# opencb/hpg-variant

Measured on AMD Instinct MI355X. Metric: variants/s chi2 assoc, higher is better.
Workload: dtype u8

## Files before the change

hpg-variant_amd/csrc/hpgv_capi.hip:

```cpp
#include "hpgv_internal.h"
#include <cstdlib>

extern "C" {

const char *hpgv_version(void) { return "hpgv-mi355x 0.1 (gfx950)"; }

int hpgv_device_count(void) {
    int n = 0;
    if (hipGetDeviceCount(&n) != hipSuccess) return -1;
    return n;
}

const char *hpgv_last_error(const hpgv_ctx *ctx) { return ctx ? ctx->err.c_str() : g_create_error.c_str(); }

static void read_environment(hpgv_ctx *ctx) {
    auto num = [](const char *name, long lo, long hi, long *out) { const char *e = getenv(name); if (e && *e) { long v = atol(e); *out = v < lo ? lo : v > hi ? hi : v; } };
    num("HPGV_BATCH_COPY", 0, 1, &ctx->batch_copy);
    num("HPGV_BATCH_FUSED", 0, 1, &ctx->batch_fused);
    num("HPGV_STATS_ALL2", 0, 1, &ctx->stats_all2);
    num("HPGV_ASSOC_ROWS", 0, 1, &ctx->assoc_rows);
    num("HPGV_PINNED_NONCOHERENT", 0, 1, &ctx->pinned_noncoherent);
    num("HPGV_VMM_TRACE", 0, 1, &ctx->vmm_trace);
    num("HPGV_DECODE_TILES", 0, 1, &ctx->decode_tiles);
#ifdef HPGV_ABLATION
// ... 45 lines not shown
        return rc;
    }
    *out = ctx;
    return HPGV_OK;
}

int hpgv_create_multi(const int *device_ids, int n_devices, hpgv_ctx **out) {
    if (!out) return fail(nullptr, HPGV_ERR_INVALID, "out is NULL");
    *out = nullptr;
    if (!device_ids || n_devices < 1 || n_devices > 64) return fail(nullptr, HPGV_ERR_INVALID, "hpgv_create_multi needs 1..64 device ids");
    hpgv_ctx *g = new (std::nothrow) hpgv_ctx();
    if (!g) return fail(nullptr, HPGV_ERR_NOMEM, "out of host memory");
    for (int i = 0; i < n_devices; ++i) {
        hpgv_ctx *m = nullptr;
        const int rc = hpgv_create(device_ids[i], &m);
        if (rc != HPGV_OK) {
            for (hpgv_ctx *c : g->members) { c->parent = nullptr; hpgv_destroy(c); }
            g->members.clear();
            delete g;
            return rc;
        }
        m->parent = g;
        g->members.push_back(m);
    }
    g->device = g->members[0]->device;
    *out = g;
    return HPGV_OK;
}

int hpgv_group_size(const hpgv_ctx *ctx) { return !ctx ? 0 : (is_group(ctx) ? (int)ctx->members.size() : 1); }

hpgv_ctx *hpgv_group_member(hpgv_ctx *ctx, int i) {
    if (!ctx) return nullptr;
    if (!is_group(ctx)) return i == 0 ? ctx : nullptr;
    return (i >= 0 && i < (int)ctx->members.size()) ? ctx->members[(size_t)i] : nullptr;
}

int hpgv_member_device(const hpgv_ctx *ctx, int i) {
    if (!ctx) return -1;
    if (!is_group(ctx)) return i == 0 ? ctx->device : -1;
    return (i >= 0 && i < (int)ctx->members.size()) ? ctx->members[(size_t)i]->device : -1;
}

}
namespace {
void grow_release(hpgv_ctx::GrowRange &r) {
    size_t off = 0;
    for (size_t i = 0; i < r.pieces.size(); ++i) { (void)hipMemUnmap(r.base + off, r.sizes[i]); (void)hipMemRelease(r.pieces[i]); off += r.sizes[i]; }
    if (r.base) (void)hipMemAddressFree(r.base, r.reserved);
    r = hpgv_ctx::GrowRange();
}
}
extern "C" {

void hpgv_destroy(hpgv_ctx *ctx) {
    if (!ctx) return;
    if (is_group(ctx)) {
        hpgv_group_release(ctx);
        for (hpgv_ctx *m : ctx->members) { m->parent = nullptr; hpgv_destroy(m); }
        ctx->members.clear();
        delete ctx;
        return;
    }
    DeviceGuard g(ctx->device);
    (void)hipDeviceSynchronize();
    if (ctx->d_mendel_male) (void)hipFree(ctx->d_mendel_male);
    if (ctx->d_sg_chunks) (void)hipFree(ctx->d_sg_chunks);
    if (ctx->d_group_of_col) (void)hipFree(ctx->d_group_of_col);
    if (ctx->d_cond) (void)hipFree(ctx->d_cond);
    for (Layout *L : {&ctx->assoc, &ctx->tdt, &ctx->stats, &ctx->sgroups, &ctx->mendel})
        if (L->d_col_of_pos) (void)hipFree(L->d_col_of_pos);
    ctx->tdt_plan.release();
    if (ctx->d_lf_base) (void)hipFree(ctx->d_lf_base);
    if (ctx->d_thr) (void)hipFree(ctx->d_thr);
    if (ctx->d_sink) (void)hipFree(ctx->d_sink);
    if (ctx->d_crc_tab) (void)hipFree(ctx->d_crc_tab);
    for (auto *t : ctx->tok_scratch) {
        if (t->d_blocks) (void)hipFree(t->d_blocks);
        if (t->d_line_off) (void)hipFree(t->d_line_off);
        if (t->d_extra) (void)hipFree(t->d_extra);
        delete t;
    }
    ctx->tok_scratch.clear();
    for (auto &r : ctx->grow) grow_release(r);
    ctx->grow.clear();
    hpgv_epi_release(ctx->epi);
    for (Slot *s : ctx->slots) {
        for (int i = 0; i < 8; ++i) if (s->buf[i]) (void)hipFree(s->buf[i]);
        if (s->h_res) (void)hipHostFree(s->h_res);
        if (s->cnt_buf) (void)hipFree(s->cnt_buf);
        if (s->stream) (void)hipStreamDestroy(s->stream);
        delete s;
    }
    for (int i = 0; i < 4; ++i) if (ctx->ev[i]) (void)hipEventDestroy(ctx->ev[i]);
    delete ctx;
}

#ifdef HPGV_ABLATION
#define HPGV_SHIPPED_ONLY(ok, what)
#else
#define HPGV_SHIPPED_ONLY(ok, what) if (!(ok)) return fail(ctx, HPGV_ERR_UNSUPPORTED, what ": that form is an ablation build's (-DHPGV_ABLATION, tools/build_ablation.py)");
#endif

int hpgv_set_option(hpgv_ctx *ctx, const char *key, long value) {
    if (is_group(ctx) && key && !strcmp(key, "group_self_exchange")) { ctx->group_self_exchange = value ? 1 : 0; return HPGV_OK; }
    GROUP_ALL(ctx, hpgv_set_option(m_, key, value))
    if (!ctx || !key) return HPGV_ERR_INVALID;
    if (!strcmp(key, "row_align")) {
        if (value < 16 || (value & (value - 1))) return fail(ctx, HPGV_ERR_INVALID, "row_align must be a power of two >= 16");
        if (ctx->assoc.set || ctx->tdt.set || ctx->stats.set)
            return fail(ctx, HPGV_ERR_STATE, "row_align must be set before the cohort");
        ctx->row_align = value;
    } else if (!strcmp(key, "row_pad")) {
        if (value < 0 || value % 16 || value > 65536) return fail(ctx, HPGV_ERR_INVALID, "row_pad must be a multiple of 16 in [0, 65536]");
        if (ctx->assoc.set || ctx->tdt.set || ctx->stats.set)
            return fail(ctx, HPGV_ERR_STATE, "row_pad must be set before the cohort");
        ctx->row_pad = value;
    } else if (!strcmp(key, "variants_per_wave")) {
        if (value < 1 || value > 1024) return fail(ctx, HPGV_ERR_INVALID, "variants_per_wave out of range");
        ctx->vpw = value;
    } else if (!strcmp(key, "nontemporal")) {
        HPGV_SHIPPED_ONLY(value != 0, "nontemporal = 0")
        ctx->nontemporal = value ? 1 : 0;
    } else if (!strcmp(key, "profile")) {
        ctx->profile = value ? 1 : 0;
    } else if (!strcmp(key, "scan_unroll")) {
        if (value != 4 && value != 8 && value != 10 && value != 12 && value != 16)
            return fail(ctx, HPGV_ERR_INVALID, "scan_unroll must be one of 4, 8, 10, 12, 16");
        HPGV_SHIPPED_ONLY(value == 4, "scan_unroll other than 4")
        ctx->scan_unroll = value;
    } else if (!strcmp(key, "pipeline")) {
        HPGV_SHIPPED_ONLY(value != 0, "pipeline = 0")
        ctx->pipeline = value ? 1 : 0;
    } else if (!strcmp(key, "fisher_cut_exp")) {
        if (value < 12 || value > 300) return fail(ctx, HPGV_ERR_INVALID, "fisher_cut_exp must be in [12, 300]");
        ctx->fisher_cut_exp = value;
    } else if (!strcmp(key, "epi_complete")) {
        ctx->epi_complete = value ? 1 : 0;
    } else if (!strcmp(key, "epi_triples_mfma")) {
        ctx->epi_triples_mfma = value ? 1 : 0;
    } else if (!strcmp(key, "epi_pairs_mfma")) {
        ctx->epi_pairs_mfma = value ? 1 : 0;
    } else if (!strcmp(key, "epi_triples_1pass")) {
        if (value < 0 || value > 2) return fail(ctx, HPGV_ERR_INVALID, "epi_triples_1pass must be 0 (two passes), 1 (the cells nine at a time) or 2 (one pass, one wave per SIMD)");
        HPGV_SHIPPED_ONLY(value != 2, "epi_triples_1pass = 2")
        ctx->epi_triples_1pass = value;
    } else if (!strcmp(key, "scan_lds")) {
        if (value < 0 || value > 160 * 1024) return fail(ctx, HPGV_ERR_INVALID, "scan_lds must be in [0, 163840]");
        ctx->scan_lds = value;
    } else if (!strcmp(key, "batch_copy")) {
        ctx->batch_copy = value ? 1 : 0;
    } else if (!strcmp(key, "inflate_wave")) {
        if (value < 0 || value > 4) return fail(ctx, HPGV_ERR_INVALID, "inflate_wave must be 0 (lane per block), 1 (by the number of blocks), 2 (wave per block), 4 (wave per block, several symbols per round) or 3 (lane per block, symbol tables in LDS)");
        HPGV_SHIPPED_ONLY(value == 1 || value == 4, "inflate_wave other than 1 / 4 (a wave per block, several symbols per round)")
        ctx->inflate_wave = value;
    } else if (!strcmp(key, "tokenizer_tiles")) {
        if (value < 0 || value > 2) return fail(ctx, HPGV_ERR_INVALID, "tokenizer_tiles must be 2 (one sweep), 1 (two sweeps) or 0 (line by line)");
        HPGV_SHIPPED_ONLY(value == 1, "tokenizer_tiles other than 1 (two sweeps)")
        ctx->tokenizer_tiles = value;
    } else if (!strcmp(key, "fisher_width")) {
        if (value != 64 && value != 32 && value != 16 && value != 8) return fail(ctx, HPGV_ERR_INVALID, "fisher_width must be 64, 32, 16 or 8");
        HPGV_SHIPPED_ONLY(value == 16, "fisher_width other than 16")
        ctx->fisher_width = value;
    } else if (!strcmp(key, "batch_fused")) {
        ctx->batch_fused = value ? 1 : 0;
    } else if (!strcmp(key, "pipe_waves")) {
        if (value != 4 && value != 6 && value != 8) return fail(ctx, HPGV_ERR_INVALID, "pipe_waves must be 4, 6 or 8");
        HPGV_SHIPPED_ONLY(value == 4, "pipe_waves other than 4")
        ctx->pipe_waves = value;
    } else if (!strcmp(key, "persistent")) {
        HPGV_SHIPPED_ONLY(value == 0, "persistent = 1")
        ctx->persistent = value ? 1 : 0;
    } else if (!strcmp(key, "part_aligned_loads")) {
        HPGV_SHIPPED_ONLY(value == 0, "part_aligned_loads = 1")
        ctx->part_aligned = value ? 1 : 0;
    } else if (!strcmp(key, "blocks_per_cu")) {
        if (value < 1 || value > 8) return fail(ctx, HPGV_ERR_INVALID, "blocks_per_cu must be in 1..8");
        ctx->blocks_per_cu = value;
    } else {
        return fail(ctx, HPGV_ERR_INVALID, "unknown option '%s'", key);
    }
    return HPGV_OK;
}


int hpgv_set_cohort(hpgv_ctx *ctx, const uint8_t *condition, int n_samples) {
    HPGV_ABI_TRY
    GROUP_ALL(ctx, hpgv_set_cohort(m_, condition, n_samples))
    if (!ctx) return HPGV_ERR_INVALID;
    if (!condition || n_samples < 0) return fail(ctx, HPGV_ERR_INVALID, "bad cohort arguments");
    DeviceGuard g(ctx->device);
    int nA = 0, nU = 0;
    for (int j = 0; j < n_samples; ++j) {
        if (condition[j] == HPGV_COND_AFFECTED) nA++;
        else if (condition[j] == HPGV_COND_UNAFFECTED) nU++;
    }
    size_t segA = round_up((size_t)nA, 16), segU = round_up((size_t)nU, 16);
    size_t pitch = round_up(segA + segU, (size_t)ctx->row_align) + (size_t)ctx->row_pad;
    if (pitch == 0) pitch = (size_t)ctx->row_align;
    if (!pitch_supported(pitch)) return fail(ctx, HPGV_ERR_UNSUPPORTED, "cohort of %d samples exceeds the row-length limit", n_samples);
    Layout &L = ctx->assoc;
    L.n_samples = n_samples;
    L.pitch = pitch;
    L.col_of_pos.assign(pitch, -1);
    size_t a = 0, u = segA;
    for (int j = 0; j < n_samples; ++j) {
        if (condition[j] == HPGV_COND_AFFECTED) L.col_of_pos[a++] = j;
        else if (condition[j] == HPGV_COND_UNAFFECTED) L.col_of_pos[u++] = j;
    }
    ctx->nA = nA; ctx->nU = nU; ctx->chunksA = (int)(segA / 16);
    {
        std::vector<uint8_t> cond(round_up((size_t)n_samples, 16) + 16, (uint8_t)HPGV_COND_OTHER);
        for (int j = 0; j < n_samples; ++j) cond[(size_t)j] = condition[j] == HPGV_COND_AFFECTED ? 1 : condition[j] == HPGV_COND_UNAFFECTED ? 0 : 2;
        if (ctx->cond_cap < cond.size()) {
            if (ctx->d_cond) { (void)hipFree(ctx->d_cond); ctx->d_cond = nullptr; ctx->cond_cap = 0; }
            HIPCHK(ctx, hipMalloc(&ctx->d_cond, cond.size()));
            ctx->cond_cap = cond.size();
        }
        HIPCHK(ctx, hipMemcpy(ctx->d_cond, cond.data(), cond.size(), hipMemcpyHostToDevice));
    }
    return upload_layout(ctx, L);
    HPGV_ABI_CATCH(ctx)
}

int hpgv_assoc_layout(const hpgv_ctx *ctx, int *n_affected, int *n_unaffected, size_t *pitch) {
    ctx = first_member(ctx);
    if (!ctx) return HPGV_ERR_INVALID;
    if (!ctx->assoc.set) return fail(ctx, HPGV_ERR_STATE, "hpgv_set_cohort has not been called");
    if (n_affected) *n_affected = ctx->nA;
    if (n_unaffected) *n_unaffected = ctx->nU;
    if (pitch) *pitch = ctx->assoc.pitch;
    return HPGV_OK;
}

int hpgv_set_logfact(hpgv_ctx *ctx, const double *table, size_t n) {
    GROUP_ALL(ctx, hpgv_set_logfact(m_, table, n))
    if (!ctx) return HPGV_ERR_INVALID;
    if (!table || n == 0) return fail(ctx, HPGV_ERR_INVALID, "empty log-factorial table");
    DeviceGuard g(ctx->device);
    ctx->n_lf = 0;
    if (ctx->cap_lf < n) {
        if (ctx->d_lf_base) { (void)hipFree(ctx->d_lf_base); ctx->d_lf_base = nullptr; ctx->d_lf = nullptr; ctx->cap_lf = 0; }
        HIPCHK(ctx, hipMalloc(&ctx->d_lf_base, (n + 4) * sizeof(double)));
        HIPCHK(ctx, hipMemset(ctx->d_lf_base, 0, (n + 4) * sizeof(double)));
        ctx->d_lf = ctx->d_lf_base + 2;
        ctx->cap_lf = n;
// ... 427 lines not shown
```

hpg-variant_amd/csrc/hpgv_internal.h:

```cpp
#pragma once
#include "../../include/hpgv.h"
#include "hpgv_kernels.h"
#include "hpgv_tdt_stats_kernels.h"
#include "hpgv_epi_kernels.h"

#include <hip/hip_runtime.h>
#include <cctype>

#include <algorithm>
#include <atomic>
#include <cmath>
#include <cstdarg>
#include <cstdio>
#include <cstring>
#include <mutex>
#include <new>
#include <string>
#include <vector>

namespace { thread_local std::string g_create_error; }

struct Layout {
    bool set = false;
    int n_samples = 0;
// ... 5 lines not shown
};

struct Slot {
    bool busy = false;
    hipStream_t stream = nullptr;
    void *buf[8] = {nullptr, nullptr, nullptr, nullptr, nullptr, nullptr, nullptr, nullptr};
    size_t cap[8] = {0, 0, 0, 0, 0, 0, 0, 0};
    void *h_res = nullptr;
    void *d_res = nullptr;
    size_t res_cap = 0;
    void *cnt_buf = nullptr;
    size_t cnt_cap = 0;
};

struct Staged {
    const uint8_t *d_raw = nullptr;
    size_t raw_pitch = 0;
    const uint8_t *d_laid = nullptr;
    int which = 0;
    const uint8_t *d_isx = nullptr;
    int n = 0;
    size_t out_stride = 0;
    bool text = false;
};

struct EpiState {
    bool have_data = false, have_folds = false;
    int V = 0, nA = 0, nU = 0, num_folds = 0, W = 0, V_alloc = 0, n_chunks = 0;
    uint8_t *d_data = nullptr;
    uint32_t *d_planes = nullptr;
    uint32_t rev_off = 0;
    hpgv_epi_rank_info rank_info{};
    uint32_t *d_marg = nullptr;
    bool complete = false;
    hpgv::EpiChunk *d_chunks = nullptr;
    uint32_t *d_chunk_cls = nullptr;
    hpgv::EpiFold *d_folds = nullptr;
    uint32_t *d_group_w0 = nullptr;
    std::vector<int32_t> group_size;
    hpgv::EpiCand *d_cand = nullptr;
    hpgv::EpiCand3 *d_cand3 = nullptr;
    size_t cand3_cap = 0;
    unsigned *d_cand_count = nullptr;
    unsigned cand_cap = 0;
    double *d_thr = nullptr;
    unsigned *d_tile_base = nullptr;
    size_t tile_base_cap = 0;
};

struct hpgv_ctx {
    std::vector<hpgv_ctx *> members;
    hpgv_ctx *parent = nullptr;
    struct GroupState *grp = nullptr;
    long group_self_exchange = 0;
    std::atomic<unsigned> deal_next{0};
    std::atomic<int> in_flight{0};
    int device = 0;
    mutable std::string err;
    std::mutex mu;
    long row_align = 16;
    long row_pad = 0;
    long vpw = 2;
    long nontemporal = 1;
    long profile = 0;
    std::mutex alias_mu;
    std::vector<std::pair<const char *, const char *>> text_alias;
    struct TextTiles { const char *d_text, *d_base; const void *d_tiles; uint64_t n_tiles; };
    std::vector<TextTiles> text_tiles;
    struct TextHeld { const char *host_text; Slot *slot; const char *d_text; const unsigned long long *d_line_off; int n_lines; };
    std::vector<TextHeld> text_held;
    long part_aligned = 0;
    long scan_unroll = 4;
    long persistent = 0;
    long blocks_per_cu = 8;
    long pipeline = 1;
    long pipe_waves = 4;
    long fisher_cut_exp = 22;
    long epi_complete = 1;
    long epi_pairs_mfma = 1;
    long epi_triples_mfma = 1;
    long epi_triples_1pass = 1;
    long scan_lds = 0;
    long fisher_width = 16;
    long inflate_wave = 1;
    long tokenizer_tiles = 1;
    long batch_copy = 0;
    long batch_fused = 1;
    long batch_lds_max = 65536;
    long stats_all2 = 1;
    long assoc_rows = 1;
    long pinned_noncoherent = 0;
    long vmm_trace = 0;
    long decode_tiles = 1;
#ifdef HPGV_ABLATION
    long stats_rows = 0, stats_bs = 0, stats_debug = 0;
    long fisher_lds = 0;
    long inflate_lds_pad = 0, inflate_wave_wgs = 0, inflate_lane_wgs = 0;
#endif
    int n_cus = 256;
    Layout assoc;
    int nA = 0, nU = 0, chunksA = 0;
    uint8_t *d_cond = nullptr;
    size_t cond_cap = 0;
    Layout tdt;
    hpgv::TdtPlan tdt_plan;
    Layout stats;
    Layout sgroups;
    std::vector<uint32_t> sg_off;
    std::vector<int> sg_size;
    int32_t *d_sg_chunks = nullptr;
    size_t sg_chunks_cap = 0;
    uint8_t *d_group_of_col = nullptr;
    size_t group_of_col_cap = 0;
    bool all_grouped = false;
    Layout mendel;
    int mendel_trios = 0, mendel_pchunks = 0;
    hpgv::MendelLuts mendel_luts{};
    uint8_t *d_mendel_male = nullptr;
    double *d_lf = nullptr;
    double *d_lf_base = nullptr;
    size_t n_lf = 0;
    size_t cap_lf = 0;
    uint32_t *d_thr = nullptr;
    size_t thr_cap = 0;
    hipEvent_t ev[4] = {nullptr, nullptr, nullptr, nullptr};
    bool have_scan_ev = false, have_stats_ev = false;
    std::vector<Slot *> slots;
    uint32_t *d_sink = nullptr;
    uint32_t *d_crc_tab = nullptr;
    struct TokScratch {
        hipStream_t stream = nullptr;
        int *d_blocks = nullptr; size_t blocks_cap = 0;
        unsigned long long *d_line_off = nullptr; size_t line_cap = 0;
        void *d_extra = nullptr; size_t extra_cap = 0;
    };
    std::mutex tok_mu;
    std::vector<TokScratch *> tok_scratch;
    struct GrowRange { char *base = nullptr; size_t reserved = 0, committed = 0; std::vector<hipMemGenericAllocationHandle_t> pieces; std::vector<size_t> sizes; };
    std::vector<GrowRange> grow;
    double filt_min_maf = -1.0, filt_max_missing = -1.0;
    long filt_max_mendel = -1;
    double filt_min_dom = -1.0, filt_min_rec = -1.0;
    std::mutex epi_mu;
    EpiState epi;
};

namespace {

[[maybe_unused]] int fail(const hpgv_ctx *ctx, int code, const char *fmt, ...) {
    char buf[512];
    va_list ap;
    va_start(ap, fmt);
    vsnprintf(buf, sizeof buf, fmt, ap);
    va_end(ap);
    if (ctx) {
        ctx->err = buf;
        if (ctx->parent) {
            std::lock_guard<std::mutex> lk(ctx->parent->mu);
            ctx->parent->err = buf;
        }
    } else g_create_error = buf;
    return code;
}

#define HPGV_ABI_TRY try {
#define HPGV_ABI_CATCH(ctx)                                                                         \
    } catch (const std::bad_alloc &) { return fail(ctx, HPGV_ERR_NOMEM, "out of host memory"); }     \
      catch (...) { return fail(ctx, HPGV_ERR_INVALID, "unexpected C++ exception inside the engine"); }

inline bool is_group(const hpgv_ctx *c) { return c && !c->members.empty(); }
inline hpgv_ctx *first_member(hpgv_ctx *c) { return is_group(c) ? c->members[0] : c; }
inline const hpgv_ctx *first_member(const hpgv_ctx *c) { return is_group(c) ? c->members[0] : c; }
struct Dealt {
    hpgv_ctx *m;
    explicit Dealt(hpgv_ctx *g) {
        const unsigned n = (unsigned)g->members.size(), start = g->deal_next.fetch_add(1u, std::memory_order_relaxed) % n;
        m = g->members[start];
        int best = m->in_flight.load(std::memory_order_relaxed);
        for (unsigned k = 1; k < n && best > 0; ++k) {
            hpgv_ctx *c = g->members[(start + k) % n];
            const int f = c->in_flight.load(std::memory_order_relaxed);
            if (f < best) { best = f; m = c; }
        }
        m->in_flight.fetch_add(1, std::memory_order_relaxed);
    }
    ~Dealt() { m->in_flight.fetch_sub(1, std::memory_order_relaxed); }
};
#define GROUP_ALL(ctx, CALL)                                                                \
    if (is_group(ctx)) {                                                                    \
        for (hpgv_ctx *m_ : (ctx)->members) { const int rc_ = CALL; if (rc_) return rc_; }  \
        return HPGV_OK;                                                                     \
    }
#define GROUP_DEAL(ctx, CALL)                                                               \
    if (is_group(ctx)) { Dealt d_(ctx); hpgv_ctx *m_ = d_.m; return CALL; }
#define GROUP_DEAL_TEXT(ctx, text, CALL)                                                    \
    if (is_group(ctx)) {                                                                    \
        if (hpgv_ctx *m_ = alias_owner(ctx, text)) return CALL;                             \
        Dealt d_(ctx); hpgv_ctx *m_ = d_.m; return CALL;                                    \
    }

#define HIPCHK(ctx, call)                                                                   \
    do {                                                                                    \
        hipError_t e_ = (call);                                                             \
        if (e_ != hipSuccess)                                                               \
            return fail(ctx, HPGV_ERR_HIP, "%s failed: %s (%s:%d)", #call,                  \
                        hipGetErrorString(e_), __FILE__, __LINE__);                         \
    } while (0)

struct DeviceGuard {
    int prev = -1;
    bool changed = false;
    explicit DeviceGuard(int dev) {
        if (hipGetDevice(&prev) == hipSuccess && prev != dev) {
            changed = (hipSetDevice(dev) == hipSuccess);
        }
    }
    ~DeviceGuard() { if (changed) (void)hipSetDevice(prev); }
};

[[maybe_unused]] size_t round_up(size_t x, size_t a) { return (x + a - 1) / a * a; }
// ... 99 lines not shown
```

hpg-variant_amd/csrc/hpgv_kernels.h:

```cpp
#pragma once
#include <hip/hip_runtime.h>
#include <stdint.h>

namespace hpgv {

__device__ __forceinline__ uint32_t nib_nonzero(uint32_t x) {
    uint32_t y = x | (x << 1);
    y = y | (y << 2);
    return y & 0x88888888u;
}
__device__ __forceinline__ uint32_t nib_not_f(uint32_t x) { return nib_nonzero(~x); }

__device__ __forceinline__ int wave_sum(int v) {
    v += __builtin_amdgcn_update_dpp(0, v, 0xB1, 0xF, 0xF, true);
    v += __builtin_amdgcn_update_dpp(0, v, 0x4E, 0xF, 0xF, true);
    v += __builtin_amdgcn_update_dpp(0, v, 0x141, 0xF, 0xF, true);
    v += __builtin_amdgcn_update_dpp(0, v, 0x140, 0xF, 0xF, true);
    return __builtin_amdgcn_readlane(v, 0) + __builtin_amdgcn_readlane(v, 16) +
           __builtin_amdgcn_readlane(v, 32) + __builtin_amdgcn_readlane(v, 48);
}

template <bool NT>
__device__ __forceinline__ uint4 load16(const uint4 *p);
template <bool NT>
// ... 280 lines not shown
}
template <int W> __device__ __forceinline__ double sub_sum_f64(double v) {
#pragma unroll
    for (int off = W / 2; off > 0; off >>= 1) v += __shfl_xor(v, off);
    return v;
}
template <int W> __device__ __forceinline__ double sub_first_f64(double v, int lane) { return __shfl(v, lane & ~(W - 1)); }

template <int W>
__device__ __forceinline__ void fisher_boundaries(const FisherTab &T, double thr , int L1, int R1, int L2, int R2, int lane,
                                                  int *xL, int *xR) {
    const int sl = sub_lane<W>(lane);
    while (R1 - L1 > W || R2 - L2 > W) {
        const bool go1 = R1 - L1 > W, go2 = R2 - L2 > W;
        const int step1 = (R1 - L1 + W - 1) / W, step2 = (R2 - L2 + W - 1) / W;
        const int x1 = L1 + sl * step1, x2 = L2 + sl * step2;
        const double v1 = (go1 && x1 < R1) ? T.e(x1) : 0.0;
        const double v2 = (go2 && x2 < R2) ? T.e(x2) : 0.0;
        if (go1) {
            const int j = __builtin_popcountll(sub_ballot<W>(x1 < R1 && v1 <= thr, lane));
            const int xj = L1 + j * step1;
            const int nL = (j == 0) ? L1 : L1 + (j - 1) * step1 + 1, nR = (j == W || xj >= R1) ? R1 : xj;
            L1 = nL; R1 = nR;
        }
        if (go2) {
            const int j = __builtin_popcountll(sub_ballot<W>(x2 < R2 && v2 > thr, lane));
            const int xj = L2 + j * step2;
            const int nL = (j == 0) ? L2 : L2 + (j - 1) * step2 + 1, nR = (j == W || xj >= R2) ? R2 : xj;
            L2 = nL; R2 = nR;
        }
    }
    const int x1 = L1 + sl, x2 = L2 + sl;
    const double v1 = x1 < R1 ? T.e(x1) : 0.0, v2 = x2 < R2 ? T.e(x2) : 0.0;
    *xL = L1 + __builtin_popcountll(sub_ballot<W>(x1 < R1 && v1 <= thr, lane));
    *xR = L2 + __builtin_popcountll(sub_ballot<W>(x2 < R2 && v2 > thr, lane));
}

template <int W>
__device__ __forceinline__ double fisher_tails(const FisherTab &T, int xL, int xR, int lo, int hi, int lane, double rel_cut) {
    const int sl = sub_lane<W>(lane);
    double partL = 0.0, partR = 0.0, cutL = 0.0, cutR = 0.0;
    bool onL = true, onR = true;
    for (int k = 0; onL || onR; ++k) {
        const int firstL = xL - 1 - 2 * W * k, firstR = xR + 2 * W * k;
        if (firstL < lo) onL = false;
        if (firstR > hi) onR = false;
        const int a = firstL - 2 * sl, b = firstR + 2 * sl;
        double eL0 = -2000.0, eL1 = -2000.0, eR0 = -2000.0, eR1 = -2000.0;
        if (onL && a >= lo) { double lo_e, hi_e; T.e2(a - 1, &lo_e, &hi_e); eL0 = hi_e; if (a - 1 >= lo) eL1 = lo_e; }
        if (onR && b <= hi) { double lo_e, hi_e; T.e2(b, &lo_e, &hi_e); eR0 = lo_e; if (b + 1 <= hi) eR1 = hi_e; }
        const double sL0 = fisher_exp(eL0, T.xt), sL1 = fisher_exp(eL1, T.xt), sR0 = fisher_exp(eR0, T.xt), sR1 = fisher_exp(eR1, T.xt);
        partL += sL0 + sL1; partR += sR0 + sR1;
        if (k == 0) { cutL = rel_cut * sub_first_f64<W>(sL0, lane); cutR = rel_cut * sub_first_f64<W>(sR0, lane); }
        if (onL && sub_ballot<W>(sL0 > cutL || sL1 > cutL, lane) == 0ull) onL = false;
        if (onR && sub_ballot<W>(sR0 > cutR || sR1 > cutR, lane) == 0ull) onR = false;
    }
    return sub_sum_f64<W>(partL + partR);
}

template <int W>
__device__ __forceinline__ bool fisher_boundary_windows(const FisherTab &T, double thr , int mode, int obs, int lane,
                                                        int *L1, int *R1, int *L2, int *R2) {
    const int sl = sub_lane<W>(lane);
    const int g1 = obs <= mode ? obs + 1 : 2 * mode - obs + 1, g2 = obs <= mode ? 2 * mode - obs : obs;
    int w1 = g1 - W / 2, w2 = g2 - W / 2;
    w1 = w1 > *R1 - W ? *R1 - W : w1; w1 = w1 < *L1 ? *L1 : w1;
    w2 = w2 > *R2 - W ? *R2 - W : w2; w2 = w2 < *L2 ? *L2 : w2;
    const int x1 = w1 + sl, x2 = w2 + sl;
    const bool in1 = x1 < *R1, in2 = x2 < *R2;
    const double v1 = in1 ? T.e(x1) : 0.0, v2 = in2 ? T.e(x2) : 0.0;
    const int n1 = __builtin_popcountll(sub_ballot<W>(in1, lane)), n2 = __builtin_popcountll(sub_ballot<W>(in2, lane));
    const int c1 = __builtin_popcountll(sub_ballot<W>(in1 && v1 <= thr, lane)), c2 = __builtin_popcountll(sub_ballot<W>(in2 && v2 > thr, lane));
    bool ok = true;
    if (c1 == 0 && w1 > *L1) { *R1 = w1; ok = false; }
    else if (c1 == n1 && w1 + n1 < *R1) { *L1 = w1 + n1; ok = false; }
    else { *L1 = w1 + c1; *R1 = w1 + c1; }
    if (c2 == 0 && w2 > *L2) { *R2 = w2; ok = false; }
    else if (c2 == n2 && w2 + n2 < *R2) { *L2 = w2 + n2; ok = false; }
    else { *L2 = w2 + c2; *R2 = w2 + c2; }
    return ok;
}

template <int W>
__device__ __forceinline__ double fisher_sub(int a, int b, int c, int d, const double *__restrict__ lf,
                                             const double *exp_tab , double rel_cut, int lane) {
    const int sl = sub_lane<W>(lane);
    const int r1 = a + b, r2 = c + d, c1 = a + c, nn = r1 + r2;
    const int lo = (c1 - r2) > 0 ? (c1 - r2) : 0;
    const int hi = r1 < c1 ? r1 : c1;
    FisherTab T;
    T.lf = lf; T.xt = exp_tab; T.r1 = r1; T.c1 = c1; T.d0 = r2 - c1;
    T.konst = lf[r1] + lf[r2] + lf[c1] + lf[nn - c1] - lf[nn];
    const double thr = T.e(a) + 9.9999995000000333e-08;
    double sum;
    if (hi - lo < 8 * W) {
        double part = 0.0;
        for (int x = lo + sl; x <= hi; x += W) {
            const double ex = T.e(x);
            if (ex <= thr) part += fisher_exp(ex, exp_tab);
        }
        sum = sub_sum_f64<W>(part);
    } else {
        const double prod = (double)(r1 + 1) * (double)(c1 + 1), den = (double)(nn + 2);
        double md = __builtin_floor(prod / den);
        const double rem = __builtin_fma(-md, den, prod);
        md += rem >= den ? 1.0 : (rem < 0.0 ? -1.0 : 0.0);
        int mode = (int)md;
        mode = mode < lo ? lo : (mode > hi ? hi : mode);
        int L1 = lo, R1 = mode + 1, L2 = mode + 1, R2 = hi + 1, xL, xR;
        if (fisher_boundary_windows<W>(T, thr, mode, a, lane, &L1, &R1, &L2, &R2)) { xL = L1; xR = L2; }
        else fisher_boundaries<W>(T, thr, L1, R1, L2, R2, lane, &xL, &xR);
        sum = fisher_tails<W>(T, xL, xR, lo, hi, lane, rel_cut);
    }
    return sum > 1.0 ? 1.0 : sum;
}

__device__ __forceinline__ double fisher_wave(int a, int b, int c, int d, const double *__restrict__ lf,
                                              const double *exp_tab , double rel_cut, int lane) {
    return fisher_sub<64>(a, b, c, d, lf, exp_tab, rel_cut, lane);
}

template <int W>
__global__ __launch_bounds__(256) void k_assoc_fisher(const int4 *__restrict__ counts, int n,
                                                      const double *__restrict__ lf,
                                                      double *__restrict__ odds,
                                                      double *__restrict__ pval, double rel_cut) {
    __shared__ double exp_tab[64];
    if (threadIdx.x < 64) exp_tab[threadIdx.x] = k_exp2_j64[threadIdx.x];
    __syncthreads();
    const int lane = threadIdx.x & 63;
    constexpr int PER_WAVE = 64 / W;
    const long wave = (long)blockIdx.x * (blockDim.x >> 6) + (threadIdx.x >> 6);
    const long v = wave * PER_WAVE + lane / W;
    if (v >= n) return;
    const int4 c4 = counts[v];
    const int a = c4.x, b = c4.y, c = c4.z, d = c4.w;
    const double p = fisher_sub<W>(a, b, c, d, lf, exp_tab, rel_cut, lane);
    if (sub_lane<W>(lane) == 0) {
        odds[v] = assoc_odds(a, b, c, d);
        pval[v] = p;
    }
}

__host__ __device__ __forceinline__ uint64_t splitmix64(uint64_t x) {
    x ^= x >> 30; x *= 0xbf58476d1ce4e5b9ULL;
    x ^= x >> 27; x *= 0x94d049bb133111ebULL;
    x ^= x >> 31;
    return x;
}
#define HPGV_SYNTH_SEED 0x4850475631ULL

static __global__ void k_synth_thresholds(uint64_t v0, int n, uint32_t *__restrict__ thr) {
    const int i = blockIdx.x * blockDim.x + threadIdx.x;
    if (i >= n) return;
    const uint64_t v = v0 + (uint64_t)i;
    const uint64_t h = splitmix64(HPGV_SYNTH_SEED ^ 0xA11E1EULL ^ v);
    const double u = (double)(h >> 11) * (1.0 / 9007199254740992.0);
    const double q = 0.05 + 0.45 * u;
    const uint32_t t_miss = 167772u;
    const double rest = (double)(16777216u - t_miss);
    const double omq = 1.0 - q;
    const double p00 = omq * omq;
    const double p01 = 2.0 * q * omq;
    const uint32_t t00 = t_miss + (uint32_t)floor(p00 * rest);
    const uint32_t t01 = t00 + (uint32_t)floor(p01 * rest);
    thr[3 * i + 0] = t_miss; thr[3 * i + 1] = t00; thr[3 * i + 2] = t01;
}

__device__ __forceinline__ uint32_t synth_gt(uint64_t vterm, uint64_t s, uint32_t tm, uint32_t t0,
                                             uint32_t t1) {
    const uint32_t r = (uint32_t)(splitmix64(vterm + s) >> 40);
    return (r < tm) ? 0xFFu : (r < t0) ? 0x00u : (r < t1) ? 0x01u : 0x11u;
}

enum { RECODE_NONE = 0, RECODE_TDT = 1, RECODE_STATS = 2, RECODE_MENDEL = 3, RECODE_EPI = 4 };

constexpr uint32_t TDT_F_UNUSABLE = 0x80u, TDT_M_UNUSABLE = 0x20u;
constexpr uint32_t TDT_C_INVALID = 4u;

__host__ __device__ __forceinline__ uint32_t tdt_parent_class(uint32_t g, uint32_t unusable) {
    const uint32_t a1 = g >> 4, a2 = g & 0xFu;
    if (a1 == 0xFu || a2 == 0xFu) return unusable;
    if (a1 && !a2) return unusable;
    if (!a1 && !a2) return 0u;
    if (!a1) return 1u;
    return (a1 == a2) ? 2u : 3u;
}
__host__ __device__ __forceinline__ uint32_t tdt_child_class(uint32_t g) {
    const uint32_t a1 = g >> 4, a2 = g & 0xFu;
    if (a1 == 0xFu || a2 == 0xFu) return TDT_C_INVALID;
    if (!a1 && !a2) return 0u;
    if (!a1) return 1u;
    if (!a2) return 2u;
    return 3u;
}
__host__ __device__ __forceinline__ uint32_t stats_flags(uint32_t g) {
    const uint32_t a1 = g >> 4, a2 = g & 0xFu;
    uint32_t f = 0;
    if (g == 0x00u) f |= 1u; else if (g == 0x01u) f |= 2u; else if (g == 0x10u) f |= 4u; else if (g == 0x11u) f |= 8u;
    if (a1 == 0xFu || a2 == 0xFu) f |= 0x10u;
    if (a1 == 0xFu && a2 == 0xFu) f |= 0x20u;
    if (!(f & 0xFu)) {
        if (a1 == 0u || a2 == 0u) f |= 0x40u;
        if (a1 == 1u || a2 == 1u) f |= 0x80u;
    }
    return f;
}

__host__ __device__ __forceinline__ uint32_t mendel_class(uint32_t g) {
    const uint32_t a1 = g >> 4, a2 = g & 0xFu;
    if (a1 == 0xFu || a2 == 0xFu) return 3u;
    if (!a1 && !a2) return 0u;
    return (a1 && a2) ? 2u : 1u;
}

__device__ __forceinline__ uint32_t recode_byte(uint32_t g, int mode, int p16, int pos, bool is_pad) {
    if (mode == RECODE_TDT) {
        if (p16 <= 0 || pos >= 3 * p16) return g;
        if (pos < p16) return tdt_parent_class(g, TDT_F_UNUSABLE);
        if (pos < 2 * p16) return tdt_parent_class(g, TDT_M_UNUSABLE);
        return tdt_child_class(g);
    }
    if (mode == RECODE_STATS) return is_pad ? 0u : stats_flags(g);
    if (mode == RECODE_MENDEL) return mendel_class(g);
    if (mode == RECODE_EPI) {
        const uint32_t a1 = g >> 4, a2 = g & 0xFu;
// ... 109 lines not shown
```

hpg-variant_amd/csrc/hpgv_scan_capi.hip:

```cpp
#include "hpgv_internal.h"
#include <type_traits>
#include "hpgv_inherit_kernels.h"

namespace {

unsigned scan_blocks(const hpgv_ctx *ctx, int n_variants) {
    const long waves = ((long)n_variants + ctx->vpw - 1) / ctx->vpw;
    return (unsigned)((waves + 3) / 4);
}

const char *const kAligned16 = "device buffers must be 16-byte aligned";
int scan_checks(hpgv_ctx *ctx, int n_variants, const void *d_gt, const void *d_out, uintptr_t out_mask, const char *align_text, bool *go) {
    *go = false;
    if (n_variants < 0 || (n_variants > 0 && (!d_gt || !d_out))) return fail(ctx, HPGV_ERR_INVALID, "bad scan arguments");
    if (n_variants == 0) return HPGV_OK;
    if (((uintptr_t)d_gt & 15) || ((uintptr_t)d_out & out_mask)) return fail(ctx, HPGV_ERR_INVALID, "%s", align_text);
    *go = true;
    return HPGV_OK;
}

template <typename F>
void launch_nt(const hpgv_ctx *ctx, F &&f) {
    if (ctx->nontemporal) f(std::true_type{}); else f(std::false_type{});
}
// ... 131 lines not shown
    const int vpw = (int)ctx->vpw;
    unsigned blocks = scan_blocks(ctx, n_variants);
    if (ctx->persistent) {
        const unsigned cap = (unsigned)(ctx->n_cus * ctx->blocks_per_cu);
        const unsigned need = (unsigned)(((long)n_variants + 3) / 4);
        blocks = need < cap ? need : cap;
    }
    hipStream_t st = (hipStream_t)stream;
    const uint8_t *gt = d_gt;
    int4 *out = (int4 *)d_counts;
    const int cA = ctx->chunksA, ch = L.chunks;
    const size_t pitch = L.pitch;
#define HPGV_LAUNCH_PIPE(NT, U, W)                                                                \
    hipLaunchKernelGGL((hpgv::k_assoc_scan_pipe<NT, U, W>), dim3(blocks), dim3(256), 0, st, gt, pitch, \
                       n_variants, cA, ch, d_is_x, out, vpw)
#ifndef HPGV_ABLATION
    return launch_profiled(ctx, st, 0, [&] { HPGV_LAUNCH_PIPE(true, 4, 4); });
#else
#define HPGV_LAUNCH_ASSOC(NT, U, S)                                                              \
    hipLaunchKernelGGL((hpgv::k_assoc_scan<NT, U, S>), dim3(blocks), dim3(256), 0, st, gt, pitch, \
                       n_variants, cA, ch, d_is_x, out, vpw)
#define HPGV_DISPATCH_U(NT, S)                                                                   \
    switch (ctx->scan_unroll) {                                                                  \
        case 4: HPGV_LAUNCH_ASSOC(NT, 4, S); break;                                              \
        case 10: HPGV_LAUNCH_ASSOC(NT, 10, S); break;                                            \
        case 12: HPGV_LAUNCH_ASSOC(NT, 12, S); break;                                            \
        case 16: HPGV_LAUNCH_ASSOC(NT, 16, S); break;                                            \
        default: HPGV_LAUNCH_ASSOC(NT, 8, S); break;                                             \
    }
#define HPGV_PIPE_W(NT, U)                                                                       \
    do {                                                                                         \
        if (ctx->pipe_waves == 8) { HPGV_LAUNCH_PIPE(NT, U, 8); }                                \
        else if (ctx->pipe_waves == 6) { HPGV_LAUNCH_PIPE(NT, U, 6); }                           \
        else { HPGV_LAUNCH_PIPE(NT, U, 4); }                                                     \
    } while (0)
    if (ctx->pipeline && !ctx->persistent)
        return launch_profiled(ctx, st, 0, [&] {
            if (ctx->nontemporal) {
                if (ctx->scan_unroll <= 4) HPGV_PIPE_W(true, 4); else HPGV_PIPE_W(true, 5);
            } else {
                if (ctx->scan_unroll <= 4) HPGV_PIPE_W(false, 4); else HPGV_PIPE_W(false, 5);
            }
        });
    return launch_profiled(ctx, st, 0, [&] {
        if (ctx->nontemporal) {
            if (ctx->persistent) { HPGV_DISPATCH_U(true, true) } else { HPGV_DISPATCH_U(true, false) }
        } else {
            if (ctx->persistent) { HPGV_DISPATCH_U(false, true) } else { HPGV_DISPATCH_U(false, false) }
        }
    });
#undef HPGV_DISPATCH_U
#undef HPGV_PIPE_W
#undef HPGV_LAUNCH_ASSOC
#endif
#undef HPGV_LAUNCH_PIPE
}

int hpgv_assoc_chisq_dev(hpgv_ctx *ctx, const int32_t *d_counts, int n_variants, double *d_odds,
                         double *d_chisq, double *d_p, void *stream) {
    ctx = first_member(ctx);
    if (!ctx) return HPGV_ERR_INVALID;
    if (n_variants < 0 || (n_variants > 0 && (!d_counts || !d_odds || !d_chisq || !d_p)))
        return fail(ctx, HPGV_ERR_INVALID, "bad chisq arguments");
    if (n_variants == 0) return HPGV_OK;
    DeviceGuard g(ctx->device);
    hipStream_t st = (hipStream_t)stream;
    return launch_profiled(ctx, st, 1, [&] {
        hipLaunchKernelGGL(hpgv::k_assoc_chisq, dim3((n_variants + 255) / 256), dim3(256), 0, st,
                           (const int4 *)d_counts, n_variants, d_odds, d_chisq, d_p);
    });
}

int hpgv_assoc_fisher_dev(hpgv_ctx *ctx, const int32_t *d_counts, int n_variants, double *d_odds,
                          double *d_p, void *stream) {
    ctx = first_member(ctx);
    if (!ctx) return HPGV_ERR_INVALID;
    if (n_variants < 0 || (n_variants > 0 && (!d_counts || !d_odds || !d_p)))
        return fail(ctx, HPGV_ERR_INVALID, "bad fisher arguments");
    if (const int rc = logfact_check(ctx)) return rc;
    if (n_variants == 0) return HPGV_OK;
    DeviceGuard g(ctx->device);
    hipStream_t st = (hipStream_t)stream;
    const double cut = pow(10.0, -(double)ctx->fisher_cut_exp);
    return launch_profiled(ctx, st, 1, [&] {
        const long per_block = 4 * (64 / ctx->fisher_width);
        const unsigned blocks = (unsigned)(((long)n_variants + per_block - 1) / per_block);
#ifdef HPGV_ABLATION
        const unsigned pad = (unsigned)ctx->fisher_lds;
        if (ctx->fisher_width == 64)
            hipLaunchKernelGGL(hpgv::k_assoc_fisher<64>, dim3(blocks), dim3(256), pad, st, (const int4 *)d_counts, n_variants, ctx->d_lf, d_odds, d_p, cut);
        else if (ctx->fisher_width == 8)
            hipLaunchKernelGGL(hpgv::k_assoc_fisher<8>, dim3(blocks), dim3(256), pad, st, (const int4 *)d_counts, n_variants, ctx->d_lf, d_odds, d_p, cut);
        else if (ctx->fisher_width == 32)
            hipLaunchKernelGGL(hpgv::k_assoc_fisher<32>, dim3(blocks), dim3(256), pad, st, (const int4 *)d_counts, n_variants, ctx->d_lf, d_odds, d_p, cut);
        else
#else
        const unsigned pad = 0u;
#endif
            hipLaunchKernelGGL(hpgv::k_assoc_fisher<16>, dim3(blocks), dim3(256), pad, st, (const int4 *)d_counts, n_variants, ctx->d_lf, d_odds, d_p, cut);
    });
}


int hpgv_tdt_scan_dev(hpgv_ctx *ctx, const uint8_t *d_gt, int n_variants, const uint8_t *d_is_x,
                      int32_t *d_tu, void *stream) {
    ctx = first_member(ctx);
    if (!ctx) return HPGV_ERR_INVALID;
    if (!ctx->tdt.set) return fail(ctx, HPGV_ERR_STATE, "hpgv_set_families has not been called");
    bool go;
    if (const int rc = scan_checks(ctx, n_variants, d_gt, d_tu, 7, "device buffers must be aligned", &go); rc || !go) return rc;
    DeviceGuard g(ctx->device);
    hipStream_t st = (hipStream_t)stream;
    return launch_profiled(ctx, st, 0, [&] {
        ctx->tdt_plan.launch_scan(d_gt, ctx->tdt.pitch, n_variants, d_is_x, (int2 *)d_tu,
                                  (int)ctx->vpw, ctx->nontemporal != 0, st);
    });
}

int hpgv_tdt_stats_dev(hpgv_ctx *ctx, const int32_t *d_tu, int n_variants, double *d_odds,
                       double *d_chisq, double *d_p, void *stream) {
    ctx = first_member(ctx);
    if (!ctx) return HPGV_ERR_INVALID;
    if (n_variants < 0 || (n_variants > 0 && (!d_tu || !d_odds || !d_chisq || !d_p)))
        return fail(ctx, HPGV_ERR_INVALID, "bad tdt stats arguments");
    if (n_variants == 0) return HPGV_OK;
    DeviceGuard g(ctx->device);
    hipStream_t st = (hipStream_t)stream;
    return launch_profiled(ctx, st, 1, [&] {
        hipLaunchKernelGGL(hpgv::k_tdt_stats, dim3((n_variants + 255) / 256), dim3(256), 0, st,
                           (const int2 *)d_tu, n_variants, d_odds, d_chisq, d_p);
    });
}


static int stats_scan(hpgv_ctx *ctx, const Layout &L, const uint8_t *d_gt, int n_variants, uint32_t off, int chunks, size_t lds,
                      int32_t *d_counts8, hipStream_t st) {
    bool go;
    if (const int rc = scan_checks(ctx, n_variants, d_gt, d_counts8, 15, kAligned16, &go); rc || !go) return rc;
    DeviceGuard g(ctx->device);
    const int vpw = (int)ctx->vpw;
    const unsigned blocks = scan_blocks(ctx, n_variants);
    return launch_profiled(ctx, st, 0, [&] {
        launch_nt(ctx, [&](auto NT) {
            constexpr bool nt = decltype(NT)::value;
            if (ctx->pipeline)
                hipLaunchKernelGGL((hpgv::k_stats_scan_hs<nt>), dim3(blocks), dim3(256), nt ? lds : 0, st, d_gt, L.pitch, n_variants, off, chunks, (int4 *)d_counts8, vpw);
            else
                hipLaunchKernelGGL((hpgv::k_stats_scan<nt, kScanUnroll>), dim3(blocks), dim3(256), 0, st, d_gt, L.pitch, n_variants, off, chunks, (int4 *)d_counts8, vpw);
        });
    });
}

int hpgv_stats_scan_dev(hpgv_ctx *ctx, const uint8_t *d_gt, int n_variants, int32_t *d_counts8, void *stream) {
    ctx = first_member(ctx);
    if (!ctx) return HPGV_ERR_INVALID;
    if (!ctx->stats.set) return fail(ctx, HPGV_ERR_STATE, "hpgv_set_stats_cohort has not been called");
    const Layout &L = ctx->stats;
    const size_t scan_lds = ctx->scan_lds > 0 ? (size_t)ctx->scan_lds : (L.pitch >= 6656 ? (size_t)49152 : (size_t)0);
    return stats_scan(ctx, L, d_gt, n_variants, 0u, L.chunks, scan_lds, d_counts8, (hipStream_t)stream);
}

int hpgv_stats_scan_group_dev(hpgv_ctx *ctx, const uint8_t *d_gt, int n_variants, int group, int32_t *d_counts8, void *stream) {
    ctx = first_member(ctx);
    if (!ctx) return HPGV_ERR_INVALID;
    if (!ctx->sgroups.set) return fail(ctx, HPGV_ERR_STATE, "hpgv_set_stats_groups has not been called");
    if (group < 0 || (size_t)group >= ctx->sg_off.size()) return fail(ctx, HPGV_ERR_INVALID, "group %d out of range", group);
// ... 168 lines not shown
```

Before: 137.8 million.

## Bin Fisher exact tests by tail length and run tails in sorted order

Splits the Fisher exact test into a plan pass and a tails pass. The plan pass computes each variant's tail boundaries and iteration counts. A histogram, prefix-scan and scatter then group variants by tail length, and a final kernel sums the tails in that order. The goal is to reduce wave divergence and load imbalance, since sub-waves would otherwise wait on the longest table. The cost is three extra kernel launches, a scratch buffer and a single-block scan.

Result: no change. 136.6 million, median of 2 (-0.9%).

```diff
diff --git a/hpg-variant_amd/csrc/hpgv_capi.hip b/hpg-variant_amd/csrc/hpgv_capi.hip
--- a/hpg-variant_amd/csrc/hpgv_capi.hip
+++ b/hpg-variant_amd/csrc/hpgv_capi.hip
@@ -151,6 +151,11 @@
         delete t;
     }
     ctx->tok_scratch.clear();
+    for (auto *f : ctx->fisher_scratch) {
+        if (f->d_buf) (void)hipFree(f->d_buf);
+        delete f;
+    }
+    ctx->fisher_scratch.clear();
     for (auto &r : ctx->grow) grow_release(r);
     ctx->grow.clear();
     hpgv_epi_release(ctx->epi);
@@ -231,6 +236,8 @@
         if (value != 64 && value != 32 && value != 16 && value != 8) return fail(ctx, HPGV_ERR_INVALID, "fisher_width must be 64, 32, 16 or 8");
         HPGV_SHIPPED_ONLY(value == 16, "fisher_width other than 16")
         ctx->fisher_width = value;
+    } else if (!strcmp(key, "fisher_binned")) {
+        ctx->fisher_binned = value ? 1 : 0;
     } else if (!strcmp(key, "batch_fused")) {
         ctx->batch_fused = value ? 1 : 0;
     } else if (!strcmp(key, "pipe_waves")) {
diff --git a/hpg-variant_amd/csrc/hpgv_internal.h b/hpg-variant_amd/csrc/hpgv_internal.h
--- a/hpg-variant_amd/csrc/hpgv_internal.h
+++ b/hpg-variant_amd/csrc/hpgv_internal.h
@@ -111,6 +111,7 @@
     long epi_triples_1pass = 1;
     long scan_lds = 0;
     long fisher_width = 16;
+    long fisher_binned = 1;
     long inflate_wave = 1;
     long tokenizer_tiles = 1;
     long batch_copy = 0;
@@ -165,6 +166,9 @@
     };
     std::mutex tok_mu;
     std::vector<TokScratch *> tok_scratch;
+    struct FisherScratch { hipStream_t stream = nullptr; void *d_buf = nullptr; size_t cap = 0; };
+    std::mutex fisher_mu;
+    std::vector<FisherScratch *> fisher_scratch;
     struct GrowRange { char *base = nullptr; size_t reserved = 0, committed = 0; std::vector<hipMemGenericAllocationHandle_t> pieces; std::vector<size_t> sizes; };
     std::vector<GrowRange> grow;
     double filt_min_maf = -1.0, filt_max_missing = -1.0;
diff --git a/hpg-variant_amd/csrc/hpgv_kernels.h b/hpg-variant_amd/csrc/hpgv_kernels.h
--- a/hpg-variant_amd/csrc/hpgv_kernels.h
+++ b/hpg-variant_amd/csrc/hpgv_kernels.h
@@ -386,6 +386,30 @@
 }
 
 template <int W>
+__device__ __forceinline__ double fisher_short(const FisherTab &T, double thr , int lo, int hi, int sl) {
+    double part = 0.0;
+    for (int x = lo + sl; x <= hi; x += W) {
+        const double ex = T.e(x);
+        if (ex <= thr) part += fisher_exp(ex, T.xt);
+    }
+    return sub_sum_f64<W>(part);
+}
+
+template <int W>
+__device__ __forceinline__ void fisher_ends(const FisherTab &T, double thr , int obs, int nn , int lo, int hi, int lane,
+                                            int *xL, int *xR) {
+    const double prod = (double)(T.r1 + 1) * (double)(T.c1 + 1), den = (double)(nn + 2);
+    double md = __builtin_floor(prod / den);
+    const double rem = __builtin_fma(-md, den, prod);
+    md += rem >= den ? 1.0 : (rem < 0.0 ? -1.0 : 0.0);
+    int mode = (int)md;
+    mode = mode < lo ? lo : (mode > hi ? hi : mode);
+    int L1 = lo, R1 = mode + 1, L2 = mode + 1, R2 = hi + 1;
+    if (fisher_boundary_windows<W>(T, thr, mode, obs, lane, &L1, &R1, &L2, &R2)) { *xL = L1; *xR = L2; }
+    else fisher_boundaries<W>(T, thr, L1, R1, L2, R2, lane, xL, xR);
+}
+
+template <int W>
 __device__ __forceinline__ double fisher_sub(int a, int b, int c, int d, const double *__restrict__ lf,
                                              const double *exp_tab , double rel_cut, int lane) {
     const int sl = sub_lane<W>(lane);
@@ -398,22 +422,10 @@
     const double thr = T.e(a) + 9.9999995000000333e-08;
     double sum;
     if (hi - lo < 8 * W) {
-        double part = 0.0;
-        for (int x = lo + sl; x <= hi; x += W) {
-            const double ex = T.e(x);
-            if (ex <= thr) part += fisher_exp(ex, exp_tab);
-        }
-        sum = sub_sum_f64<W>(part);
+        sum = fisher_short<W>(T, thr, lo, hi, sl);
     } else {
-        const double prod = (double)(r1 + 1) * (double)(c1 + 1), den = (double)(nn + 2);
-        double md = __builtin_floor(prod / den);
-        const double rem = __builtin_fma(-md, den, prod);
-        md += rem >= den ? 1.0 : (rem < 0.0 ? -1.0 : 0.0);
-        int mode = (int)md;
-        mode = mode < lo ? lo : (mode > hi ? hi : mode);
-        int L1 = lo, R1 = mode + 1, L2 = mode + 1, R2 = hi + 1, xL, xR;
-        if (fisher_boundary_windows<W>(T, thr, mode, a, lane, &L1, &R1, &L2, &R2)) { xL = L1; xR = L2; }
-        else fisher_boundaries<W>(T, thr, L1, R1, L2, R2, lane, &xL, &xR);
+        int xL, xR;
+        fisher_ends<W>(T, thr, a, nn, lo, hi, lane, &xL, &xR);
         sum = fisher_tails<W>(T, xL, xR, lo, hi, lane, rel_cut);
     }
     return sum > 1.0 ? 1.0 : sum;
@@ -446,6 +458,164 @@
     }
 }
 
+constexpr int FISHER_BINS = 64;
+constexpr int FISHER_NOT_PLANNED = 255;
+struct alignas(16) FisherPlan { int xL, xR, kL, kR; };
+
+__device__ __forceinline__ FisherTab fisher_tab(int a, int b, int c, int d, const double *__restrict__ lf, const double *exp_tab ,
+                                                int *lo, int *hi) {
+    const int r1 = a + b, r2 = c + d, c1 = a + c, nn = r1 + r2;
+    *lo = (c1 - r2) > 0 ? (c1 - r2) : 0;
+    *hi = r1 < c1 ? r1 : c1;
+    FisherTab T;
+    T.lf = lf; T.xt = exp_tab; T.r1 = r1; T.c1 = c1; T.d0 = r2 - c1;
+    T.konst = lf[r1] + lf[r2] + lf[c1] + lf[nn - c1] - lf[nn];
+    return T;
+}
+
+template <int W>
+__device__ __forceinline__ void fisher_tail_turns(const FisherTab &T, int xL, int xR, int lo, int hi, double ln_cut, int lane, int *kL, int *kR) {
+    const int sl = sub_lane<W>(lane);
+    const int maxL = (xL - lo + 2 * W - 1) / (2 * W), maxR = (hi - xR + 1 + 2 * W - 1) / (2 * W);
+    const double cL = T.e(maxL > 0 ? xL - 1 : lo) + ln_cut, cR = T.e(maxR > 0 ? xR : hi) + ln_cut;
+    int nL = maxL, nR = maxR;
+    bool goL = maxL > 1, goR = maxR > 1;
+    for (int base = 1; goL || goR; base += W) {
+        const int k = base + sl;
+        const bool inL = goL && k < maxL, inR = goR && k < maxR;
+        const double vL = inL ? T.e(xL - 1 - 2 * W * k) : 0.0;
+        const double vR = inR ? T.e(xR + 2 * W * k) : 0.0;
+        const uint64_t bL = sub_ballot<W>(inL && vL <= cL, lane), bR = sub_ballot<W>(inR && vR <= cR, lane);
+        if (goL) {
+            if (bL) { nL = base + __builtin_ctzll(bL); goL = false; }
+            else if (base + W >= maxL) goL = false;
+        }
+        if (goR) {
+            if (bR) { nR = base + __builtin_ctzll(bR); goR = false; }
+            else if (base + W >= maxR) goR = false;
+        }
+    }
+    *kL = nL; *kR = nR;
+}
+
+template <int W>
+__global__ __launch_bounds__(256) void k_assoc_fisher_plan(const int4 *__restrict__ counts, int n, int per_block,
+                                                           const double *__restrict__ lf,
+                                                           double *__restrict__ odds, double *__restrict__ pval, double ln_cut,
+                                                           FisherPlan *__restrict__ plan, uint8_t *__restrict__ bin_of,
+                                                           uint32_t *__restrict__ hist) {
+    __shared__ double exp_tab[64];
+    __shared__ uint32_t cnt[FISHER_BINS];
+    if (threadIdx.x < 64) exp_tab[threadIdx.x] = k_exp2_j64[threadIdx.x];
+    if (threadIdx.x < FISHER_BINS) cnt[threadIdx.x] = 0u;
+    __syncthreads();
+    const int lane = threadIdx.x & 63, sl = sub_lane<W>(lane);
+    constexpr int PER_WAVE = 64 / W;
+    const long begin = (long)blockIdx.x * per_block;
+    const long end = begin + per_block < n ? begin + per_block : n;
+    for (long v = begin + (threadIdx.x >> 6) * PER_WAVE + lane / W; v < end; v += 4 * PER_WAVE) {
+        const int4 c4 = counts[v];
+        const int a = c4.x, b = c4.y, c = c4.z, d = c4.w;
+        int lo, hi;
+        const FisherTab T = fisher_tab(a, b, c, d, lf, exp_tab, &lo, &hi);
+        const double thr = T.e(a) + 9.9999995000000333e-08;
+        if (hi - lo < 8 * W) {
+            const double sum = fisher_short<W>(T, thr, lo, hi, sl);
+            if (sl == 0) { pval[v] = sum > 1.0 ? 1.0 : sum; bin_of[v] = (uint8_t)FISHER_NOT_PLANNED; }
+        } else {
+            FisherPlan P;
+            fisher_ends<W>(T, thr, a, a + b + c + d, lo, hi, lane, &P.xL, &P.xR);
+            fisher_tail_turns<W>(T, P.xL, P.xR, lo, hi, ln_cut, lane, &P.kL, &P.kR);
+            if (sl == 0) {
+                const int K = P.kL > P.kR ? P.kL : P.kR;
+                const int bin = FISHER_BINS - 1 - (K < FISHER_BINS - 1 ? K : FISHER_BINS - 1);
+                plan[v] = P;
+                bin_of[v] = (uint8_t)bin;
+                atomicAdd(&cnt[bin], 1u);
+            }
+        }
+        if (sl == 0) odds[v] = assoc_odds(a, b, c, d);
+    }
+    __syncthreads();
+    if (threadIdx.x < FISHER_BINS) hist[(size_t)threadIdx.x * gridDim.x + blockIdx.x] = cnt[threadIdx.x];
+}
+
+static __global__ __launch_bounds__(1024) void k_assoc_fisher_bins(uint32_t *__restrict__ hist, int n_entries, uint32_t *__restrict__ total) {
+    __shared__ uint32_t part[1024];
+    const int t = threadIdx.x;
+    const int per = (n_entries + 1023) / 1024;
+    const int lo = t * per < n_entries ? t * per : n_entries, hi = lo + per < n_entries ? lo + per : n_entries;
+    uint32_t s = 0u;
+    for (int i = lo; i < hi; ++i) s += hist[i];
+    part[t] = s;
+    __syncthreads();
+    for (int off = 1; off < 1024; off <<= 1) {
+        const uint32_t add = t >= off ? part[t - off] : 0u;
+        __syncthreads();
+        part[t] += add;
+        __syncthreads();
+    }
+    uint32_t run = part[t] - s;
+    for (int i = lo; i < hi; ++i) { const uint32_t c = hist[i]; hist[i] = run; run += c; }
+    if (t == 1023) *total = part[1023];
+}
+
+static __global__ __launch_bounds__(64) void k_assoc_fisher_scatter(const uint8_t *__restrict__ bin_of, int n, int per_block,
+                                                                    const uint32_t *__restrict__ base, uint32_t *__restrict__ list) {
+    const int lane = threadIdx.x;
+    static_assert(FISHER_BINS == 64, "one lane per bin");
+    uint32_t next = base[(size_t)lane * gridDim.x + blockIdx.x];
+    const long begin = (long)blockIdx.x * per_block;
+    const long end = begin + per_block < n ? begin + per_block : n;
+    for (long v0 = begin; v0 < end; v0 += 64) {
+        const long v = v0 + lane;
+        const int bin = v < end ? (int)bin_of[v] : FISHER_NOT_PLANNED;
+        uint64_t todo = __ballot(bin != FISHER_NOT_PLANNED);
+        while (todo) {
+            const int bb = __shfl(bin, (int)__builtin_ctzll(todo));
+            const uint64_t same = __ballot(bin == bb);
+            const uint32_t slot = __shfl(next, bb);
+            if (bin == bb) list[slot + (uint32_t)__builtin_popcountll(same & ((1ull << lane) - 1ull))] = (uint32_t)v;
+            if (lane == bb) next += (uint32_t)__builtin_popcountll(same);
+            todo &= ~same;
+        }
+    }
+}
+
+template <int W>
+__global__ __launch_bounds__(256) void k_assoc_fisher_tails(const int4 *__restrict__ counts, const double *__restrict__ lf,
+                                                            const FisherPlan *__restrict__ plan, const uint32_t *__restrict__ list,
+                                                            const uint32_t *__restrict__ total, double *__restrict__ pval) {
+    __shared__ double exp_tab[64];
+    constexpr int PER_WAVE = 64 / W;
+    const uint32_t n_planned = *total;
+    if ((uint64_t)blockIdx.x * (4 * PER_WAVE) >= n_planned) return;
+    if (threadIdx.x < 64) exp_tab[threadIdx.x] = k_exp2_j64[threadIdx.x];
+    __syncthreads();
+    const int lane = threadIdx.x & 63, sl = sub_lane<W>(lane);
+    const uint64_t i = ((uint64_t)blockIdx.x * 4 + (threadIdx.x >> 6)) * PER_WAVE + lane / W;
+    if (i >= n_planned) return;
+    const uint32_t v = list[i];
+    const int4 c4 = counts[v];
+    const FisherPlan P = plan[v];
+    int lo, hi;
+    const FisherTab T = fisher_tab(c4.x, c4.y, c4.z, c4.w, lf, exp_tab, &lo, &hi);
+    const int K = P.kL > P.kR ? P.kL : P.kR;
+    double partL = 0.0, partR = 0.0;
+    for (int k = 0; k < K; ++k) {
+        const bool onL = k < P.kL, onR = k < P.kR;
+        const int firstL = P.xL - 1 - 2 * W * k, firstR = P.xR + 2 * W * k;
+        const int a = firstL - 2 * sl, b = firstR + 2 * sl;
+        double eL0 = -2000.0, eL1 = -2000.0, eR0 = -2000.0, eR1 = -2000.0;
+        if (onL && a >= lo) { double lo_e, hi_e; T.e2(a - 1, &lo_e, &hi_e); eL0 = hi_e; if (a - 1 >= lo) eL1 = lo_e; }
+        if (onR && b <= hi) { double lo_e, hi_e; T.e2(b, &lo_e, &hi_e); eR0 = lo_e; if (b + 1 <= hi) eR1 = hi_e; }
+        const double sL0 = fisher_exp(eL0, T.xt), sL1 = fisher_exp(eL1, T.xt), sR0 = fisher_exp(eR0, T.xt), sR1 = fisher_exp(eR1, T.xt);
+        partL += sL0 + sL1; partR += sR0 + sR1;
+    }
+    const double sum = sub_sum_f64<W>(partL + partR);
+    if (sl == 0) pval[v] = sum > 1.0 ? 1.0 : sum;
+}
+
 __host__ __device__ __forceinline__ uint64_t splitmix64(uint64_t x) {
     x ^= x >> 30; x *= 0xbf58476d1ce4e5b9ULL;
     x ^= x >> 27; x *= 0x94d049bb133111ebULL;
diff --git a/hpg-variant_amd/csrc/hpgv_scan_capi.hip b/hpg-variant_amd/csrc/hpgv_scan_capi.hip
--- a/hpg-variant_amd/csrc/hpgv_scan_capi.hip
+++ b/hpg-variant_amd/csrc/hpgv_scan_capi.hip
@@ -237,6 +237,47 @@
     DeviceGuard g(ctx->device);
     hipStream_t st = (hipStream_t)stream;
     const double cut = pow(10.0, -(double)ctx->fisher_cut_exp);
+    if (ctx->fisher_binned && ctx->fisher_width == 16) {
+        const long groups = ((long)n_variants + 15) / 16;
+        const long plan_blocks = std::min(groups, (long)ctx->n_cus * 8);
+        const int per_block = (int)((groups + plan_blocks - 1) / plan_blocks) * 16;
+        const unsigned nb = (unsigned)(((long)n_variants + per_block - 1) / per_block);
+        const size_t n_hist = (size_t)hpgv::FISHER_BINS * nb;
+        const size_t off_list = round_up((size_t)n_variants * sizeof(hpgv::FisherPlan), 256);
+        const size_t off_hist = off_list + round_up((size_t)n_variants * sizeof(uint32_t), 256);
+        const size_t off_bin = off_hist + round_up((n_hist + 1) * sizeof(uint32_t), 256);
+        const size_t need = off_bin + round_up((size_t)n_variants, 256);
+        hpgv_ctx::FisherScratch *fs = nullptr;
+        {
+            std::lock_guard<std::mutex> lk(ctx->fisher_mu);
+            for (auto *f : ctx->fisher_scratch) if (f->stream == st) fs = f;
+            if (!fs) {
+                fs = new (std::nothrow) hpgv_ctx::FisherScratch();
+                if (!fs) return fail(ctx, HPGV_ERR_NOMEM, "out of host memory");
+                fs->stream = st;
+                ctx->fisher_scratch.push_back(fs);
+            }
+        }
+        if (fs->cap < need) {
+            if (fs->d_buf) { HIPCHK(ctx, hipStreamSynchronize(st)); (void)hipFree(fs->d_buf); fs->d_buf = nullptr; fs->cap = 0; }
+            const size_t want = round_up(need + need / 4, 256);
+            HIPCHK(ctx, hipMalloc(&fs->d_buf, want));
+            fs->cap = want;
+        }
+        char *base = (char *)fs->d_buf;
+        hpgv::FisherPlan *d_plan = (hpgv::FisherPlan *)base;
+        uint32_t *d_list = (uint32_t *)(base + off_list), *d_hist = (uint32_t *)(base + off_hist), *d_total = d_hist + n_hist;
+        uint8_t *d_bin = (uint8_t *)(base + off_bin);
+        const double ln_cut = -(double)ctx->fisher_cut_exp * 2.302585092994046;
+        return launch_profiled(ctx, st, 1, [&] {
+            hipLaunchKernelGGL(hpgv::k_assoc_fisher_plan<16>, dim3(nb), dim3(256), 0, st, (const int4 *)d_counts, n_variants, per_block,
+                               ctx->d_lf, d_odds, d_p, ln_cut, d_plan, d_bin, d_hist);
+            hipLaunchKernelGGL(hpgv::k_assoc_fisher_bins, dim3(1), dim3(1024), 0, st, d_hist, (int)n_hist, d_total);
+            hipLaunchKernelGGL(hpgv::k_assoc_fisher_scatter, dim3(nb), dim3(64), 0, st, d_bin, n_variants, per_block, d_hist, d_list);
+            hipLaunchKernelGGL(hpgv::k_assoc_fisher_tails<16>, dim3((unsigned)groups), dim3(256), 0, st, (const int4 *)d_counts, ctx->d_lf,
+                               d_plan, d_list, d_total, d_p);
+        });
+    }
     return launch_profiled(ctx, st, 1, [&] {
         const long per_block = 4 * (64 / ctx->fisher_width);
         const unsigned blocks = (unsigned)(((long)n_variants + per_block - 1) / per_block);
```
